# manuelbb-upb/Morbit.jl

Hardware: AMD Instinct MI355X
Metric: RBF build+solve+eval cycles/sec (higher is better)
Workload: dtype f64

## Files before the change

morbit.jl_amd/csrc/backsolve.hip:

```cpp
#include "common.hpp"

namespace mrbf {

namespace bsolve {

constexpr int NB = 128, NTHR = 512;
typedef double v2d __attribute__((ext_vector_type(2)));
typedef double v4d __attribute__((ext_vector_type(4)));
typedef __attribute__((address_space(1))) unsigned gu32;
typedef __attribute__((address_space(1))) double gf64;
typedef __attribute__((address_space(1))) v2d gv2d;

template <int KB>
struct Shared {
    double xs[2][KB][NB];
    int ok;
};

__global__ __launch_bounds__(256) void premul_kernel(const double *__restrict__ L, int64_t lda, const double *__restrict__ linv_all,
                                                     double *__restrict__ Mbuf, int nb, unsigned *__restrict__ flags, int nflags,
                                                     unsigned long long *__restrict__ xb, int nxb) {
    for (int e = blockIdx.x * 256 + threadIdx.x; e < nflags; e += gridDim.x * 256) flags[e] = 0u;
    for (int e = blockIdx.x * 256 + threadIdx.x; e < nxb; e += gridDim.x * 256) xb[e] = ~0ull;
    const int slab = blockIdx.x & 3, t = (blockIdx.x >> 2) & 1, j = blockIdx.x >> 3;
    const int i = j + 1 + t;
    if (i >= nb) return;
    const double *A = L + (int64_t)i * NB + (int64_t)j * NB * lda;
    const double *B = linv_all + (size_t)j * NB * NB;
    double *M = Mbuf + ((size_t)j * 2 + t) * NB * NB;
    const int lane = threadIdx.x & 63, wave = threadIdx.x >> 6, l15 = lane & 15, l4 = lane >> 4;
    const int i0 = 32 * wave, j0 = 32 * slab;
    v4d acc[2][2];
#pragma unroll
    for (int a = 0; a < 2; ++a)
#pragma unroll
        for (int b = 0; b < 2; ++b) acc[a][b] = (v4d){0.0, 0.0, 0.0, 0.0};
    const double *pa = A + (i0 + l15) + (int64_t)(j0 + l4) * lda;
    const double *pb = B + (j0 + l4) + (int64_t)(j0 + l15) * NB;
    constexpr int UK = 8;
    double fa0[2][UK], fa1[2][UK], fb0[2][UK], fb1[2][UK];
    auto burst = [&](int buf) {
#pragma unroll
        for (int u = 0; u < UK; ++u) {
            fa0[buf][u] = pa[(int64_t)4 * u * lda];
            fa1[buf][u] = pa[(int64_t)4 * u * lda + 16];
            fb0[buf][u] = pb[4 * u];
            fb1[buf][u] = pb[4 * u + 16 * NB];
        }
        pa += (int64_t)4 * UK * lda;
        pb += 4 * UK;
    };
    auto mma = [&](int buf) {
#pragma unroll
        for (int u = 0; u < UK; ++u) {
            acc[0][0] = __builtin_amdgcn_mfma_f64_16x16x4f64(fa0[buf][u], fb0[buf][u], acc[0][0], 0, 0, 0);
            acc[0][1] = __builtin_amdgcn_mfma_f64_16x16x4f64(fa0[buf][u], fb1[buf][u], acc[0][1], 0, 0, 0);
            acc[1][0] = __builtin_amdgcn_mfma_f64_16x16x4f64(fa1[buf][u], fb0[buf][u], acc[1][0], 0, 0, 0);
            acc[1][1] = __builtin_amdgcn_mfma_f64_16x16x4f64(fa1[buf][u], fb1[buf][u], acc[1][1], 0, 0, 0);
        }
    };
    const int nburst = (NB - j0) / (4 * UK);
    burst(0);
    for (int b = 0; b < nburst; b += 2) {
        if (b + 1 < nburst) burst(1);
        mma(0);
        if (b + 1 >= nburst) break;
        if (b + 2 < nburst) burst(0);
        mma(1);
    }
#pragma unroll
    for (int a = 0; a < 2; ++a)
#pragma unroll
        for (int b = 0; b < 2; ++b)
#pragma unroll
            for (int r = 0; r < 4; ++r) M[(i0 + 16 * a + l4 + 4 * r) + (size_t)(j0 + 16 * b + l15) * NB] = acc[a][b][r];
}

__device__ __forceinline__ void load_tile(const double *__restrict__ T, int64_t ldt, v2d (&r)[2][8]) {
    const int lane = threadIdx.x & 63, w = threadIdx.x >> 6;
    const double *p = T + (int64_t)(16 * w + 2 * (lane >> 3)) * ldt + 2 * (lane & 7);
#pragma unroll
    for (int cc = 0; cc < 2; ++cc)
#pragma unroll
        for (int u = 0; u < 8; ++u) r[cc][u] = *(const gv2d *)(p + cc * ldt + 16 * u);
}

template <int N>
__device__ __forceinline__ double shl_lanes(double v) {
    const long long b = __double_as_longlong(v);
    const int lo = __builtin_amdgcn_update_dpp((int)b, (int)b, 0x100 + N, 0xf, 0xf, false);
    const int hi = __builtin_amdgcn_update_dpp((int)(b >> 32), (int)(b >> 32), 0x100 + N, 0xf, 0xf, false);
    return __longlong_as_double(((long long)hi << 32) | (unsigned)lo);
}

template <int KB>
__device__ __forceinline__ void tile_dot(const double (*xs)[NB], const v2d (&r)[2][8], double (&out)[2][KB]) {
    const int q = threadIdx.x & 7;
    double acc[2][KB];
#pragma unroll
    for (int cc = 0; cc < 2; ++cc)
#pragma unroll
        for (int l = 0; l < KB; ++l) acc[cc][l] = 0.0;
#pragma unroll
    for (int u = 0; u < 8; ++u) {
#pragma unroll
        for (int l = 0; l < KB; ++l) {
            const v2d x = *(const v2d *)&xs[l][16 * u + 2 * q];
#pragma unroll
            for (int cc = 0; cc < 2; ++cc) acc[cc][l] = fma(r[cc][u][1], x[1], fma(r[cc][u][0], x[0], acc[cc][l]));
        }
    }
#pragma unroll
    for (int cc = 0; cc < 2; ++cc)
#pragma unroll
        for (int l = 0; l < KB; ++l) {
            double v = acc[cc][l];
            v += shl_lanes<4>(v);
            v += shl_lanes<2>(v);
            v += shl_lanes<1>(v);
            out[cc][l] = v;
        }
}

template <int KB>
__device__ __forceinline__ void await_block(Shared<KB> &sh, double (*xs)[NB], const double *glob, int i, double spec, int backoff,
                                            unsigned *abortw, unsigned epoch, unsigned long long spin_ticks, int *status, int code) {
    const int tid = threadIdx.x;
    if (tid >= KB * NB) return;
    const gf64 *src = (const gf64 *)&glob[((size_t)i * KB + tid / NB) * NB + (tid % NB)];
    double v = spec;
    if (__double_as_longlong(v) == -1ll) v = __hip_atomic_load(src, __ATOMIC_RELAXED, __HIP_MEMORY_SCOPE_AGENT);
    unsigned spins = 0;
    unsigned long long t0 = 0;
    while (__double_as_longlong(v) == -1ll) {
        if ((++spins & 63u) == 0u) {
            if (__hip_atomic_load((const gu32 *)abortw, __ATOMIC_RELAXED, __HIP_MEMORY_SCOPE_AGENT) != 0u) {
                sh.ok = 0;
                break;
            }
            const unsigned long long now = wall_clock64();
            if (t0 == 0) t0 = now;
            if (now - t0 > spin_ticks) {
                __hip_atomic_store((gu32 *)abortw, epoch, __ATOMIC_RELAXED, __HIP_MEMORY_SCOPE_AGENT);
                *(__attribute__((address_space(1))) int *)status = code + (i & 0xff);
                sh.ok = 0;
                break;
            }
        }
        for (int b = 0; b < backoff; ++b) __builtin_amdgcn_s_sleep(8);
        v = __hip_atomic_load(src, __ATOMIC_RELAXED, __HIP_MEMORY_SCOPE_AGENT);
    }
    xs[tid / NB][tid % NB] = v;
}

__device__ __forceinline__ void lds_barrier() { asm volatile("s_waitcnt lgkmcnt(0)\n\ts_barrier" ::: "memory"); }

__device__ __forceinline__ void publish(double *dst, v2d v) {
    if (__double_as_longlong(v[0]) == -1ll) v[0] = __longlong_as_double(0x7ff8000000000000ll);
    if (__double_as_longlong(v[1]) == -1ll) v[1] = __longlong_as_double(0x7ff8000000000000ll);
    asm volatile("global_store_dwordx4 %0, %1, off sc1" ::"v"(dst), "v"(v) : "memory");
}

template <int KB>
__global__ __launch_bounds__(NTHR, 1) void backsolve_persistent_kernel(const double *__restrict__ L, int64_t lda, const double *__restrict__ linv_all,
                                                                        const double *__restrict__ Mbuf, double *__restrict__ Y, int64_t ldy, int k0,
                                                                        int nb, unsigned *flags, unsigned epoch, unsigned long long spin_ticks,
                                                                        int *status, int fault, double *__restrict__ xb, double *__restrict__ zb,
                                                                        long long *stamps) {
    __shared__ __attribute__((aligned(16))) Shared<KB> sh;
    const int p = (int)blockIdx.x >> 1;
    const bool finisher = blockIdx.x & 1;
    const int j = nb - 1 - p, tid = threadIdx.x;
    const int lane = tid & 63, col = 16 * (tid >> 6) + 2 * (lane >> 3), q = lane & 7;
    unsigned *abortw = flags + (size_t)nb * 32;
    const int na = nb - 1 - j, npm = na < 2 ? na : 2, npl = na - npm;
    if (tid == 0) sh.ok = 1;
    __syncthreads();
    const double fillv = __longlong_as_double(-1ll);
    if (!finisher) {
        double w[2][KB];
#pragma unroll
        for (int cc = 0; cc < 2; ++cc)
#pragma unroll
            for (int l = 0; l < KB; ++l) w[cc][l] = *(const gf64 *)&Y[(int64_t)(k0 + l) * ldy + (int64_t)j * NB + col + cc];
        const int nst = npl + 1;
        auto fetch = [&](int s, v2d(&r)[2][8]) {
            const double *src = s < npl ? L + (int64_t)(nb - 1 - s) * NB + (int64_t)j * NB * lda : linv_all + (size_t)j * NB * NB;
            load_tile(src, s < npl ? lda : (int64_t)NB, r);
        };
        auto look = [&](int s) {
            const int i = nb - 1 - (s < npl ? s : (npl > 0 ? npl - 1 : 0));
            const int e = tid < KB * NB ? tid : 0;
            return __hip_atomic_load((const gf64 *)&xb[((size_t)i * KB + e / NB) * NB + (e % NB)], __ATOMIC_RELAXED, __HIP_MEMORY_SCOPE_AGENT);
        };
        double spec = fillv, spec2 = fillv;
        auto step = [&](int s, const v2d(&r)[2][8]) -> bool {
            double(*xs)[NB] = sh.xs[s & 1];
            if (s < npl) {
                const int i = nb - 1 - s;
                const int backoff = (i - j - 3) < 24 ? (i - j - 3) : 24;
                await_block<KB>(sh, xs, xb, i, spec, backoff, abortw, epoch, spin_ticks, status, 0x700);
                if (stamps && tid == 0 && s == npl - 1) stamps[256 * 5 + j * 4 + 0] = (long long)wall_clock64();
            } else if (q == 0) {
#pragma unroll
                for (int l = 0; l < KB; ++l) *(v2d *)&xs[l][col] = (v2d){w[0][l], w[1][l]};
            }
            spec = spec2;
            spec2 = look(s + 2);
            if (s + 2 >= npl) spec2 = fillv;
            lds_barrier();
            if (!sh.ok) return false;
            double dsum[2][KB];
            tile_dot<KB>(xs, r, dsum);
#pragma unroll
            for (int cc = 0; cc < 2; ++cc)
#pragma unroll
                for (int l = 0; l < KB; ++l) w[cc][l] = s == npl ? dsum[cc][l] : w[cc][l] - dsum[cc][l];
            return true;
        };
        v2d t0[2][8], t1[2][8], t2[2][8];
        const int o = (3 - nst % 3) % 3, G = (nst + o) / 3;
        if (0 - o >= 0) fetch(0 - o, t0);
        if (1 - o >= 0) fetch(1 - o, t1);
        fetch(2 - o, t2);
        spec = look(0);
        if (npl == 0) spec = fillv;
        spec2 = look(1);
        if (npl <= 1) spec2 = fillv;
        int g = 0;
        if (G >= 2) {
            const int s = -o;
            if (s >= 0 && !step(s, t0)) return;
            fetch(s + 3, t0);
            if (s + 1 >= 0 && !step(s + 1, t1)) return;
            fetch(s + 4, t1);
            if (!step(s + 2, t2)) return;
            fetch(s + 5, t2);
            g = 1;
        }
        for (; g < G - 1; ++g) {
            const int s = 3 * g - o;
            if (!step(s, t0)) return;
            fetch(s + 3, t0);
            if (!step(s + 1, t1)) return;
            fetch(s + 4, t1);
            if (!step(s + 2, t2)) return;
            fetch(s + 5, t2);
        }
        {
            const int s = 3 * (G - 1) - o;
            if (s >= 0 && !step(s, t0)) return;
            if (s + 1 >= 0 && !step(s + 1, t1)) return;
            if (!step(s + 2, t2)) return;
        }
        if (stamps && tid == 0) stamps[256 * 5 + j * 4 + 1] = (long long)wall_clock64();
        if (q == 0) {
#pragma unroll
            for (int l = 0; l < KB; ++l) publish(&zb[((size_t)j * KB + l) * NB + col], (v2d){w[0][l], w[1][l]});
        }
        return;
    }
    v2d tm2[2][8], tm1[2][8];
    if (npm == 2) load_tile(Mbuf + ((size_t)j * 2 + 1) * NB * NB, NB, tm2);
    if (npm >= 1) load_tile(Mbuf + (size_t)j * 2 * NB * NB, NB, tm1);
    double acc[2][KB];
#pragma unroll
    for (int cc = 0; cc < 2; ++cc)
#pragma unroll
        for (int l = 0; l < KB; ++l) acc[cc][l] = 0.0;
    if (npm == 2) {
        await_block<KB>(sh, sh.xs[0], xb, j + 2, fillv, 1, abortw, epoch, spin_ticks, status, 0x700);
        lds_barrier();
        if (!sh.ok) return;
        if (stamps && tid == 0) stamps[256 * 5 + j * 4 + 3] = (long long)wall_clock64();
        tile_dot<KB>(sh.xs[0], tm2, acc);
    }
    v2d zj[KB];
    if (q == 0) {
        unsigned spins = 0;
        unsigned long long t0 = 0;
#pragma unroll
        for (int l = 0; l < KB; ++l) {
            const double *src = &zb[((size_t)j * KB + l) * NB + col];
            while (true) {
                v2d v;
                asm volatile("global_load_dwordx4 %0, %1, off sc1\n\ts_waitcnt vmcnt(0)" : "=v"(v) : "v"(src) : "memory");
                if (__double_as_longlong(v[0]) != -1ll && __double_as_longlong(v[1]) != -1ll) {
                    zj[l] = v;
                    break;
                }
                if ((++spins & 63u) == 0u) {
                    if (__hip_atomic_load((const gu32 *)abortw, __ATOMIC_RELAXED, __HIP_MEMORY_SCOPE_AGENT) != 0u) {
                        sh.ok = 0;
                        break;
                    }
                    const unsigned long long now = wall_clock64();
                    if (t0 == 0) t0 = now;
                    if (now - t0 > spin_ticks) {
                        __hip_atomic_store((gu32 *)abortw, epoch, __ATOMIC_RELAXED, __HIP_MEMORY_SCOPE_AGENT);
                        *(__attribute__((address_space(1))) int *)status = 0x600 + (j & 0xff);
                        sh.ok = 0;
                        break;
                    }
                }
                __builtin_amdgcn_s_sleep(2);
            }
            if (!sh.ok) break;
        }
    }
    if (stamps && tid == 0) stamps[256 * 5 + j * 4 + 2] = (long long)wall_clock64();
    double last[2][KB];
#pragma unroll
    for (int cc = 0; cc < 2; ++cc)
#pragma unroll
        for (int l = 0; l < KB; ++l) last[cc][l] = 0.0;
    if (npm >= 1) {
        if (stamps && tid == 0) stamps[256 * 4 + j] = (long long)wall_clock64();
        await_block<KB>(sh, sh.xs[1], xb, j + 1, fillv, 0, abortw, epoch, spin_ticks, status, 0x700);
        if (stamps && tid == 0) stamps[j * 4 + 0] = (long long)wall_clock64();
        lds_barrier();
        if (!sh.ok) return;
        if (stamps && tid == 0) stamps[j * 4 + 1] = (long long)wall_clock64();
        tile_dot<KB>(sh.xs[1], tm1, last);
    } else {
        lds_barrier();
        if (!sh.ok) return;
    }
    if ((fault & 1) && j == nb / 2) return;
    if (stamps && tid == 0) stamps[j * 4 + 2] = (long long)wall_clock64();
    if (q == 0) {
#pragma unroll
        for (int l = 0; l < KB; ++l) {
            const v2d v = (v2d){(zj[l][0] - acc[0][l]) - last[0][l], (zj[l][1] - acc[1][l]) - last[1][l]};
            publish(&xb[((size_t)j * KB + l) * NB + col], v);
            *(v2d *)&Y[(int64_t)(k0 + l) * ldy + (int64_t)j * NB + col] = v;
        }
    }
}

}

int backsolve_blocked(mrbf_ctx *ctx, int64_t npad, const double *L, int64_t lda, const double *linv_all, double *Y, int64_t ldy, int k);

int backsolve_persistent(mrbf_ctx *ctx, int64_t npad, const double *L, int64_t lda, const double *linv_all, double *Y, int64_t ldy, int k,
                         int *status) {
    using namespace bsolve;
    const int nb = (int)(npad / NB);
    static const int force_old = mrbf_env("MRBF_BACKSOLVE_LAUNCHES") ? atoi(mrbf_env("MRBF_BACKSOLVE_LAUNCHES")) : 0;
    const int ncu = ctx->ncu;
    if (force_old || nb < 3 || nb > ncu || (lda & 1) || (reinterpret_cast<uintptr_t>(L) & 15))
        return backsolve_blocked(ctx, npad, L, lda, linv_all, Y, ldy, k);
    unsigned *flags;
    MRBF_TRY(get_buf(ctx, S_BSOLVE_FLAGS, (size_t)(nb + 1) * 32, &flags));
    const unsigned long long spin_ticks = (unsigned long long)std::max(1, ctx->spin_ms) * 100000ull;
    const int fault = (ctx->debug_fault & 2) ? 1 : 0;
    double *xb, *Mbuf;
    MRBF_TRY(get_buf(ctx, S_BSOLVE_X, (size_t)2 * nb * 4 * NB, &xb));
    MRBF_TRY(get_buf(ctx, S_BSOLVE_M, (size_t)nb * 2 * NB * NB, &Mbuf));
    hipLaunchKernelGGL(premul_kernel, dim3((unsigned)(8 * (nb - 1))), dim3(256), 0, ctx->stream, L, lda, linv_all, Mbuf, nb, flags, (nb + 1) * 32,
                       reinterpret_cast<unsigned long long *>(xb), 2 * nb * 4 * NB);
    static const bool want_stamps = mrbf_env("MRBF_BSOLVE_STAMPS") && atoi(mrbf_env("MRBF_BSOLVE_STAMPS")) != 0;
    long long *stamps = nullptr;
    if (want_stamps) {
        static long long *dbg = nullptr;
        if (!dbg) MRBF_HIP(ctx, hipMalloc(&dbg, (size_t)256 * 9 * sizeof(long long)));
        stamps = dbg;
    }
    unsigned epoch = 0;
    for (int k0 = 0; k0 < k; k0 += 4) {
        const int kb = std::min(4, k - k0);
        ++epoch;
        if (k0 > 0) MRBF_HIP(ctx, hipMemsetAsync(xb, 0xff, (size_t)2 * nb * 4 * NB * sizeof(double), ctx->stream));
#define MRBF_BSP(KBV)                                                                                                          \
    hipLaunchKernelGGL((backsolve_persistent_kernel<KBV>), dim3((unsigned)(2 * nb)), dim3(NTHR), 0, ctx->stream, L, lda, linv_all, Mbuf, Y, ldy, k0, nb, \
                       flags, epoch, spin_ticks, status, fault, xb, xb + (size_t)nb * 4 * NB, stamps)
        if (kb == 1) MRBF_BSP(1); else if (kb == 2) MRBF_BSP(2); else if (kb == 3) MRBF_BSP(3); else MRBF_BSP(4);
#undef MRBF_BSP
    }
    MRBF_HIP(ctx, hipGetLastError());
    if (want_stamps) {
        std::vector<long long> h((size_t)256 * 9);
        MRBF_HIP(ctx, hipMemcpyAsync(h.data(), stamps, h.size() * sizeof(long long), hipMemcpyDeviceToHost, ctx->stream));
        MRBF_HIP(ctx, hipStreamSynchronize(ctx->stream));
        double seen = 0, bar = 0, dot = 0, hop = 0, late = 0;
        int cnt = 0;
        for (int j = 1; j + 2 < nb; ++j) {
            seen += (double)(h[j * 4 + 0] - h[(j + 1) * 4 + 2]);
            bar += (double)(h[j * 4 + 1] - h[j * 4 + 0]);
            dot += (double)(h[j * 4 + 2] - h[j * 4 + 1]);
            hop += (double)(h[j * 4 + 2] - h[(j + 1) * 4 + 2]);
            late += (double)(h[256 * 4 + j] - h[(j + 1) * 4 + 2]);
            ++cnt;
        }
        double a3 = 0, zt = 0, zs = 0, x2 = 0;
        int c2 = 0;
        for (int j = 2; j + 4 < nb; ++j) {
            const long long *S = &h[256 * 5 + j * 4];
            a3 += (double)(S[0] - h[(j + 3) * 4 + 2]);
            zt += (double)(S[1] - S[0]);
            zs += (double)(S[2] - S[1]);
            x2 += (double)(S[3] - h[(j + 2) * 4 + 2]);
            ++c2;
        }
        fprintf(stderr, "[backsolve stamps] streamer: x_{j+3} seen %.2f us after its publication, z_j published %.2f us later, finisher has z_j %.2f us "
                "later; finisher past x_{j+2} %.2f us after that block's publication\n", a3 / c2 / 100.0, zt / c2 / 100.0, zs / c2 / 100.0, x2 / c2 / 100.0);
        fprintf(stderr, "[backsolve stamps] nb %d: publish -> seen %.2f us, seen -> barrier %.2f us, barrier -> publish %.2f us, step %.2f us; "
                "the finisher starts polling %.2f us after the publication\n", nb, seen / cnt / 100.0, bar / cnt / 100.0, dot / cnt / 100.0,
                hop / cnt / 100.0, late / cnt / 100.0);
    }
    return 0;
}

}
```

morbit.jl_amd/csrc/solve.hip:

```cpp
#include "common.hpp"
#include "small.hpp"

namespace mrbf {

__global__ void fit_publish_kernel(const int *__restrict__ dinfo, const double *__restrict__ scal, const unsigned long long *__restrict__ dstat,
                                   int *__restrict__ hflags, double *__restrict__ hscal, unsigned long long *__restrict__ hstat) {
    const int t = threadIdx.x;
    if (t < 4) hflags[t] = dinfo[t];
    if (t >= 4 && t < 6 && scal) hscal[t - 4] = scal[t - 4];
    if (t == 6 && dstat && hstat) hstat[0] = dstat[0];
}

__global__ void fill_saddle_kernel(const double *__restrict__ Pi, int64_t n, int q, double *__restrict__ S, int64_t N) {
    const int64_t idx = (int64_t)blockIdx.x * blockDim.x + threadIdx.x;
    const int64_t tot = n * q;
    if (idx < tot) {
        const int64_t i = idx % n;
        const int t = (int)(idx / n);
        const double v = Pi[idx];
        S[i + (n + t) * N] = v;
        S[(n + t) + i * N] = v;
    } else if (idx < tot + (int64_t)q * q) {
        const int64_t r = idx - tot;
        S[(n + r % q) + (n + r / q) * N] = 0.0;
// ... 223 lines not shown
    MRBF_HIP(ctx, hipEventElapsedTime(&info->ms_solve, ctx->ev[2], ctx->ev[3]));
    return 0;
}

static int fit_small_lu(mrbf_ctx *ctx, mrbf_model *M, const double *Y, mrbf_fit_info *info) {
    smallfit::Prob P;
    double *ws, *scal;
    int *flags;
    MRBF_TRY(get_buf(ctx, S_SMALL_LU, small_lu_scratch_doubles(M->n, M->q), &ws));
    MRBF_TRY(get_buf(ctx, S_SMALL_FLAGS, (size_t)4, &flags));
    MRBF_TRY(get_buf(ctx, S_MISC, (size_t)8, &scal));
    fill_small_prob(ctx, M, Y, ws, flags, scal, nullptr, &P);
    int hflags_local[4] = {0, 0, 0, 0};
    int *hflags = ctx->hpin ? reinterpret_cast<int *>(ctx->hpin + HPIN_SMALL_FLAGS) : hflags_local;
    MRBF_HIP(ctx, hipEventRecord(ctx->ev[0], ctx->stream));
    MRBF_TRY(launch_small_lu(ctx, &P, 1, nullptr));
    MRBF_HIP(ctx, hipEventRecord(ctx->ev[1], ctx->stream));
    MRBF_HIP(ctx, hipMemcpyAsync(hflags, flags, 4 * sizeof(int), hipMemcpyDeviceToHost, ctx->stream));
    MRBF_HIP(ctx, hipStreamSynchronize(ctx->stream));
    info->factor_info = hflags[0];
    info->path = MRBF_PATH_LU;
    if (hflags[0] != 0)
        return fail(ctx, MRBF_ESINGULAR, "saddle matrix is singular (getrf info = %d, N = %lld)", hflags[0], (long long)(M->n + M->q));
    MRBF_HIP(ctx, hipEventElapsedTime(&info->ms_factor, ctx->ev[0], ctx->ev[1]));
    return 0;
}

__global__ void scale_rows_pinv_kernel(double *__restrict__ T, int N, int k, const double *__restrict__ sv) {
    const int idx = blockIdx.x * blockDim.x + threadIdx.x;
    if (idx >= N * k) return;
    const int i = idx % N;
    const double s = sv[i], cut = (double)N * 2.220446049250313e-16 * sv[0];
    T[idx] = (s > cut) ? T[idx] / s : 0.0;
}

static int fit_minnorm(mrbf_ctx *ctx, mrbf_model *M, const double *Y, mrbf_fit_info *info) {
    const int64_t n = M->n, N = n + M->q;
    const int k = M->k, q = M->q;
    const double one = 1.0, zero = 0.0;
    double *S, *B, *Pi, *U, *VT, *sv, *E, *T;
    int *dinfo;
    MRBF_TRY(get_buf(ctx, S_PHI, (size_t)N * N, &S));
    MRBF_TRY(get_buf(ctx, S_RHS, (size_t)N * k, &B));
    MRBF_TRY(get_buf(ctx, S_PI, (size_t)n * q, &Pi));
    MRBF_TRY(get_buf(ctx, S_Q1, (size_t)N * N, &U));
    MRBF_TRY(get_buf(ctx, S_W1, (size_t)N * N, &VT));
    MRBF_TRY(get_buf(ctx, S_TAU, (size_t)2 * N, &sv));
    MRBF_TRY(get_buf(ctx, S_T1, (size_t)N * k, &T));
    MRBF_TRY(get_buf(ctx, S_INFO, (size_t)4, &dinfo));
    E = sv + N;
    hipLaunchKernelGGL(rhs_from_values_kernel, dim3(nblk(N * k)), dim3(256), 0, ctx->stream, Y, n, k, B, N);
    MRBF_HIP(ctx, hipEventRecord(ctx->ev[0], ctx->stream));
    MRBF_TRY(launch_gram(ctx, ctx->gram_mode, M->C, M->Xc, M->sq, n, M->npad, M->d, M->dpad, M->kp, S, N));
    MRBF_HIP(ctx, hipEventRecord(ctx->ev[1], ctx->stream));
    MRBF_TRY(launch_poly_matrix(ctx, M->C, n, M->d, q, Pi, n));
    hipLaunchKernelGGL(fill_saddle_kernel, dim3(nblk(n * q + (int64_t)q * q)), dim3(256), 0, ctx->stream, Pi, n, q, S, N);
    MRBF_HIP(ctx, hipGetLastError());
    MRBF_BLAS(ctx, rocsolver_dgesvd(ctx->blas, rocblas_svect_all, rocblas_svect_all, (int)N, (int)N, S, (int)N, sv, U, (int)N, VT,
                                    (int)N, E, rocblas_outofplace, dinfo));
    MRBF_HIP(ctx, hipEventRecord(ctx->ev[2], ctx->stream));
    int hinfo = 0;
    MRBF_TRY(read_info(ctx, dinfo, &hinfo));
    info->factor_info = hinfo;
    info->path = MRBF_PATH_MINNORM;
    if (hinfo != 0) return fail(ctx, MRBF_ESINGULAR, "SVD of the saddle matrix did not converge (info = %d)", hinfo);
    MRBF_BLAS(ctx, rocblas_dgemm(ctx->blas, rocblas_operation_transpose, rocblas_operation_none, (int)N, k, (int)N, &one, U, (int)N,
                                 B, (int)N, &zero, T, (int)N));
    hipLaunchKernelGGL(scale_rows_pinv_kernel, dim3(nblk(N * k)), dim3(256), 0, ctx->stream, T, (int)N, k, sv);
    MRBF_BLAS(ctx, rocblas_dgemm(ctx->blas, rocblas_operation_transpose, rocblas_operation_none, (int)N, k, (int)N, &one, VT, (int)N,
                                 T, (int)N, &zero, B, (int)N));
    hipLaunchKernelGGL(scatter_solution_kernel, dim3(nblk(M->npad * k + (int64_t)q * k)), dim3(256), 0, ctx->stream, B, N, n,
                       M->npad, k, q, n, M->W, M->Wc, M->lam, B, N);
    MRBF_HIP(ctx, hipGetLastError());
    MRBF_HIP(ctx, hipEventRecord(ctx->ev[3], ctx->stream));
    MRBF_HIP(ctx, hipEventSynchronize(ctx->ev[3]));
    MRBF_HIP(ctx, hipEventElapsedTime(&info->ms_gram, ctx->ev[0], ctx->ev[1]));
    MRBF_HIP(ctx, hipEventElapsedTime(&info->ms_factor, ctx->ev[1], ctx->ev[2]));
    MRBF_HIP(ctx, hipEventElapsedTime(&info->ms_solve, ctx->ev[2], ctx->ev[3]));
    return 0;
}

int backsolve_blocked(mrbf_ctx *ctx, int64_t npad, const double *L, int64_t lda, const double *linv_all, double *Y, int64_t ldy, int k);
int backsolve_persistent(mrbf_ctx *ctx, int64_t npad, const double *L, int64_t lda, const double *linv_all, double *Y, int64_t ldy, int k,
                         int *status);
int launch_update_lower(mrbf_ctx *ctx, const double *A, int64_t lda, const double *B, int64_t ldb, double *C, int64_t ldc, int64_t nt, int K,
                        const double *cvec, double cs, int64_t cn);
int launch_pad_identity(mrbf_ctx *ctx, double *A, int64_t n, int64_t npad, int64_t ld);
int tsmm_tn(mrbf_ctx *ctx, int64_t n, int p, int r, double alpha, const double *A, int64_t lda, const double *B, int64_t ldb, double beta,
            double *C, int64_t ldc);
int symm_panel(mrbf_ctx *ctx, int64_t n, int64_t npad, int q, const double *Phi, int64_t ld, const double *Q, int64_t ldq, double *W,
               int64_t ldwo, bool const_first, double cval);

__global__ void set_rhs_rows_kernel(double *__restrict__ A, int64_t ld, int64_t npad, int xt, const double *__restrict__ B, int k) {
    const int64_t idx = (int64_t)blockIdx.x * blockDim.x + threadIdx.x;
    if (idx >= npad * xt) return;
    const int l = (int)(idx % xt);
    const int64_t i = idx / xt;
    A[(npad + l) + i * ld] = (l < k) ? B[i + (int64_t)l * npad] : 0.0;
}
__global__ void get_rhs_rows_kernel(const double *__restrict__ A, int64_t ld, int64_t npad, double *__restrict__ B, int k) {
    const int64_t idx = (int64_t)blockIdx.x * blockDim.x + threadIdx.x;
    if (idx >= npad * k) return;
    const int l = (int)(idx % k);
    const int64_t i = idx / k;
    B[i + (int64_t)l * npad] = A[(npad + l) + i * ld];
}
__global__ void xc_to_tall_kernel(const double *__restrict__ Xc, int64_t n, int d, int dpad, double *__restrict__ Tall, int64_t lt,
                                  int64_t dq) {
    const int64_t idx = (int64_t)blockIdx.x * blockDim.x + threadIdx.x;
    if (idx >= n * d) return;
    const int64_t i = idx / d;
    const int t = (int)(idx % d);
    Tall[(dq + i) + (int64_t)t * lt] = Xc[i * dpad + t];
}
__global__ void build_q1_kernel(const double *__restrict__ Tall, int64_t lt, int64_t dq, int64_t n, int64_t npad, int q,
                                double *__restrict__ Q1) {
    const int64_t idx = (int64_t)blockIdx.x * blockDim.x + threadIdx.x;
    if (idx >= npad * q) return;
    const int64_t i = idx % npad;
    const int t = (int)(idx / npad);
    double v = 0.0;
    if (i < n) v = (t == 0) ? 1.0 / sqrt((double)n) : Tall[(dq + i) + (int64_t)(t - 1) * lt];
    Q1[idx] = v;
}
__global__ void shift_from_trace_kernel(double *__restrict__ scal, double nphi0, double nmq, int *__restrict__ flags) {
    const double mu = (nphi0 - scal[0]) / nmq;
    const bool ok = mu > 0.0 && mu < 1e300;
    scal[1] = ok ? mu : 1.0;
    flags[2] = ok ? 0 : 1;
}

__global__ void build_panels_kernel(const double *__restrict__ Q1, const double *__restrict__ W, const double *__restrict__ scal,
                                    int64_t n, int64_t npad, int q, int K2, int skip, double *__restrict__ PA, double *__restrict__ PB,
                                    double *__restrict__ v0) {
    const int64_t idx = (int64_t)blockIdx.x * blockDim.x + threadIdx.x;
    if (idx >= npad * K2) return;
    const double mu = scal[1];
    const int64_t i = idx % npad;
    const int t = (int)(idx / npad);
    const int qq = q - skip;
    double a = 0.0, b = 0.0;
    if (i < n && t < 2 * qq) {
        const int tt = t % qq + skip;
        const double qv = Q1[i + (int64_t)tt * npad];
        const double vv = fma(-0.5 * mu, qv, W[i + (int64_t)tt * npad]);
        a = (t < qq) ? qv : vv;
        b = (t < qq) ? vv : qv;
    }
    PA[idx] = a;
    PB[idx] = b;
    if (skip && t == 0) v0[i] = (i < n) ? fma(-0.5 * mu, Q1[i], W[i]) : 0.0;
}
__global__ __launch_bounds__(64) void finish_lambda_kernel(double *__restrict__ T1, int q, int k, double sqrtn, const double *__restrict__ mean) {
    __shared__ double part[64];
    const int l = blockIdx.x, tid = threadIdx.x;
    if (l >= k) return;
    double acc = 0.0;
    for (int t = 1 + tid; t < q; t += 64) acc = fma(mean[t - 1], T1[t + (int64_t)l * q], acc);
    part[tid] = acc;
    __syncthreads();
    if (tid == 0) {
        double dsum = 0.0;
        for (int u = 0; u < 64; ++u) dsum += part[u];
        T1[(int64_t)l * q] = T1[(int64_t)l * q] / sqrtn - dsum;
    }
}

// ... 239 lines not shown
        if (tailq) {
            double *scratch;
            MRBF_TRY(get_buf(ctx, S_PI, tail_basis_scratch_doubles(), &scratch));
            MRBF_TRY(get_buf(ctx, S_QR_INV, (size_t)128 * 128, &LxInv));
            MRBF_TRY(launch_tail_basis(ctx, M, Y, scratch, LxInv, T1, Q1, B, builtin ? Phi : nullptr, ld, xt, dinfo));
        } else if (q > 1) {
            dq = round_up(d, 128);
            lt = dq + npad;
            MRBF_TRY(get_buf(ctx, S_PI, (size_t)lt * dq, &Tall));
            MRBF_HIP(ctx, hipMemsetAsync(Tall, 0, (size_t)lt * dq * sizeof(double), ctx->stream));
            hipLaunchKernelGGL(xc_to_tall_kernel, dim3(nblk(n * d)), dim3(256), 0, ctx->stream, M->Xc, n, d, M->dpad, Tall, lt, dq);
            MRBF_TRY(tsmm_tn(ctx, n, d, d, 1.0, Tall + dq, lt, Tall + dq, lt, 0.0, Tall, lt));
            MRBF_TRY(launch_pad_identity(ctx, Tall, d, dq, lt));
            if (dq == 128) MRBF_TRY(get_buf(ctx, S_QR_INV, (size_t)128 * 128, &LxInv));
            MRBF_TRY(potrf_blocked_tall(ctx, dq, lt, Tall, lt, dinfo + 1, LxInv, popt));
        }
        if (!tailq) hipLaunchKernelGGL(build_q1_kernel, dim3(nblk(npad * q)), dim3(256), 0, ctx->stream, Tall, lt, dq, n, npad, q, Q1);
        if (!fused) MRBF_HIP(ctx, hipMemsetAsync(Wm, 0, (size_t)npad * q * sizeof(double), ctx->stream));
        if (!tailq) {
            MRBF_TRY(tsmm_tn(ctx, n, q, k, 1.0, Q1, npad, B, npad, 0.0, T1, q));
            hipLaunchKernelGGL(sub_qt_kernel, dim3((unsigned)((n + 63) / 64)), dim3(256), 0, ctx->stream, B, npad, Q1, npad, T1, n, q, k);
            if (builtin) hipLaunchKernelGGL(set_rhs_rows_kernel, dim3(nblk(npad * xt)), dim3(256), 0, ctx->stream, Phi, ld, npad, xt, B, k);
        }
        if (side) MRBF_HIP(ctx, hipEventRecord(ctx->evx[1], ctx->stream));
    }
    ctx->stream = main_stream;
    MRBF_HIP(ctx, hipEventRecord(ctx->ev[0], ctx->stream));
    double *Wpart = nullptr, *rspart = nullptr;
    int nseg = 0;
    if (fused)
        MRBF_TRY(launch_gram_w(ctx, M, Phi, ld, &Wpart, &rspart, &nseg));
    else
        MRBF_TRY(launch_gram(ctx, ctx->gram_mode, M->C, M->Xc, M->sq, n, M->npad, M->d, M->dpad, M->kp, Phi, ld));
    MRBF_HIP(ctx, hipEventRecord(ctx->ev[1], ctx->stream));
    if (side) MRBF_HIP(ctx, hipStreamWaitEvent(ctx->stream, ctx->evx[1], 0));
    if (fused) {
        const int skip = (q > 1 && round_up(2 * (q - 1), 16) < round_up(2 * q, 16)) ? 1 : 0;
        const int K2 = (int)round_up(2 * (q - skip), 16);
        double *PA, *PB, *v0 = nullptr;
        MRBF_TRY(get_buf(ctx, S_STAGE_C, (size_t)npad * K2, &PA));
        MRBF_TRY(get_buf(ctx, S_STAGE_D, (size_t)npad * K2, &PB));
        if (skip) MRBF_TRY(get_buf(ctx, S_V0, (size_t)npad, &v0));
        MRBF_TRY(launch_projection_small(ctx, M, Wpart, rspart, nseg, LxInv, Q1, Wm, G, scal, dinfo, K2, skip, PA, PB, v0));
        MRBF_TRY(launch_update_lower(ctx, PA, npad, PB, npad, Phi, ld, npad / 128, K2, v0, 1.0 / std::sqrt((double)n), n));
    } else if (q > 0) {
        MRBF_TRY(symm_panel(ctx, n, npad, q, Phi, ld, Q1, npad, Wm, npad, true, 1.0 / std::sqrt((double)n)));
        MRBF_TRY(tsmm_tn(ctx, n, q, q, 1.0, Q1, npad, Wm, npad, 0.0, G, q));
        hipLaunchKernelGGL(trace_kernel, dim3(1), dim3(256), 0, ctx->stream, G, q, scal);
        MRBF_BLAS(ctx, rocblas_dgemm(ctx->blas, rocblas_operation_none, rocblas_operation_none, (int)n, q, q, &mhalf, Q1, (int)npad,
                                     G, q, &one, Wm, (int)npad));
        hipLaunchKernelGGL(shift_from_trace_kernel, dim3(1), dim3(1), 0, ctx->stream, scal, (double)n * M->kp.phi0,
                           (double)std::max<int64_t>(n - q, 1), dinfo);
        const int skip = (q > 1 && round_up(2 * (q - 1), 16) < round_up(2 * q, 16)) ? 1 : 0;
        const int K2 = (int)round_up(2 * (q - skip), 16);
        double *PA, *PB, *v0 = nullptr;
        MRBF_TRY(get_buf(ctx, S_STAGE_C, (size_t)npad * K2, &PA));
        MRBF_TRY(get_buf(ctx, S_STAGE_D, (size_t)npad * K2, &PB));
        if (skip) MRBF_TRY(get_buf(ctx, S_V0, (size_t)npad, &v0));
        hipLaunchKernelGGL(build_panels_kernel, dim3(nblk(npad * K2)), dim3(256), 0, ctx->stream, Q1, Wm, scal, n, npad, q, K2, skip, PA, PB, v0);
        MRBF_TRY(launch_update_lower(ctx, PA, npad, PB, npad, Phi, ld, npad / 128, K2, v0, 1.0 / std::sqrt((double)n), n));
    }
    MRBF_HIP(ctx, hipEventRecord(ctx->ev[2], ctx->stream));
    int hinfo = 0;
    double *linv_all = nullptr;
    if (builtin) {
        MRBF_TRY(get_buf(ctx, S_CHOL_WS, (size_t)npad * 128, &linv_all));
        MRBF_TRY(launch_pad_identity(ctx, Phi, n, npad, ld));
        if (q == 0) hipLaunchKernelGGL(set_rhs_rows_kernel, dim3(nblk(npad * xt)), dim3(256), 0, ctx->stream, Phi, ld, npad, xt, B, k);
        popt.xreal = k;
        popt.info_clean = true;
        MRBF_TRY(potrf_blocked_tall(ctx, npad, npad + xt, Phi, ld, dinfo, linv_all, popt));
        MRBF_HIP(ctx, hipEventRecord(ctx->ev[3], ctx->stream));
    } else {
        int *dpot;
        MRBF_TRY(get_buf(ctx, S_IPIV, (size_t)4, &dpot));
        MRBF_BLAS(ctx, rocsolver_dpotrf(ctx->blas, rocblas_fill_lower, (int)n, Phi, (int)ld, dpot));
        MRBF_HIP(ctx, hipMemcpyAsync(dinfo, dpot, sizeof(int), hipMemcpyDeviceToDevice, ctx->stream));
        MRBF_HIP(ctx, hipEventRecord(ctx->ev[3], ctx->stream));
    }
    double *T1w = nullptr;
    if (q > 0) MRBF_TRY(get_buf(ctx, S_T1W, (size_t)q * k, &T1w));
    auto solve_tail = [&](bool persistent) -> int {
        if (builtin) {
            hipLaunchKernelGGL(get_rhs_rows_kernel, dim3(nblk(npad * k)), dim3(256), 0, ctx->stream, Phi, ld, npad, B, k);
            if (persistent)
                MRBF_TRY(backsolve_persistent(ctx, npad, Phi, ld, linv_all, B, npad, k, dinfo + 3));
            else
                MRBF_TRY(backsolve_blocked(ctx, npad, Phi, ld, linv_all, B, npad, k));
        } else {
            MRBF_BLAS(ctx, rocsolver_dpotrs(ctx->blas, rocblas_fill_lower, (int)n, k, Phi, (int)ld, B, (int)npad));
        }
        static const int tail3 = mrbf_env("MRBF_TAIL3") ? atoi(mrbf_env("MRBF_TAIL3")) : 1;
        if (tail3 && q > 0 && q <= 129 && k <= 16 && (q == 1 || LxInv)) {
            const int nch = (int)(npad / 64);
            double *T2, *part;
            MRBF_TRY(get_buf(ctx, S_T2, (size_t)q * k, &T2));
            MRBF_TRY(get_buf(ctx, S_TAIL_PART, (size_t)nch * 2 * k * q, &part));
            hipLaunchKernelGGL(tail_dots_kernel, dim3((unsigned)nch), dim3(256), 0, ctx->stream, B, npad, Q1, Wm, npad, n, q, k, part);
            hipLaunchKernelGGL(tail_coeff_kernel, dim3(1), dim3(1024), 0, ctx->stream, part, nch, q, k, q > 1 ? d : 0, T1, G, fused ? 1.0 : 0.5, LxInv,
                               std::sqrt((double)n), M->mean, T2, T1w);
            hipLaunchKernelGGL(tail_apply_kernel, dim3((unsigned)nch), dim3(256), 0, ctx->stream, B, npad, Q1, npad, T2, T1w, n, M->npad, q, k, M->W,
                               M->Wc, M->lam);
            MRBF_HIP(ctx, hipGetLastError());
            return 0;
        }
        if (q > 0) {
            double *T2;
            MRBF_TRY(get_buf(ctx, S_T2, (size_t)q * k, &T2));
            MRBF_HIP(ctx, hipMemcpyAsync(T1w, T1, (size_t)q * k * sizeof(double), hipMemcpyDeviceToDevice, ctx->stream));
            MRBF_TRY(tsmm_tn(ctx, n, q, k, 1.0, Q1, npad, B, npad, 0.0, T2, q));
            hipLaunchKernelGGL(sub_qt_kernel, dim3((unsigned)((n + 63) / 64)), dim3(256), 0, ctx->stream, B, npad, Q1, npad, T2, n, q, k);
            MRBF_TRY(tsmm_tn(ctx, n, q, k, -1.0, Wm, npad, B, npad, 1.0, T1w, q));
            if (q > 1) {
                if (LxInv)
                    hipLaunchKernelGGL(apply_linv_t_kernel, dim3(1), dim3(256), 0, ctx->stream, LxInv, d, T1w + 1, (int64_t)q, k);
                else if (d <= 256)
                    hipLaunchKernelGGL(trsm_lt_small_kernel, dim3(1), dim3(256), 0, ctx->stream, Tall, lt, d, T1w + 1, (int64_t)q, k);
                else
                    MRBF_BLAS(ctx, rocblas_dtrsm(ctx->blas, rocblas_side_left, rocblas_fill_lower, rocblas_operation_transpose,
                                                 rocblas_diagonal_non_unit, d, k, &one, Tall, (int)lt, T1w + 1, q));
            }
            hipLaunchKernelGGL(finish_lambda_kernel, dim3((unsigned)k), dim3(64), 0, ctx->stream, T1w, q, k, std::sqrt((double)n), M->mean);
        }
        hipLaunchKernelGGL(scatter_solution_kernel, dim3(nblk(M->npad * k + (int64_t)q * k)), dim3(256), 0, ctx->stream, B, npad, n,
                           M->npad, k, q, (int64_t)0, M->W, M->Wc, M->lam, T1w ? T1w : B, (int64_t)q);
        MRBF_HIP(ctx, hipGetLastError());
        return 0;
    };
    MRBF_TRY(solve_tail(true));
    MRBF_HIP(ctx, hipEventRecord(ctx->ev[4], ctx->stream));
    {
        int hflags_local[4] = {0, 0, 0, 0};
        double hscal_local[2] = {0.0, 0.0};
        int *hflags = ctx->hpin ? reinterpret_cast<int *>(ctx->hpin + HPIN_FIT_FLAGS) : hflags_local;
        double *hscal = ctx->hpin ? reinterpret_cast<double *>(ctx->hpin + HPIN_FIT_SCAL) : hscal_local;
        hscal[0] = hscal[1] = 0.0;
        static const int publish = mrbf_env("MRBF_FIT_PUBLISH") ? atoi(mrbf_env("MRBF_FIT_PUBLISH")) : 1;
        if (ctx->hpin && publish) {
            unsigned long long *hstat = nullptr;
            const unsigned long long *dstat = nullptr;
            if (ctx->mega_stat_pending && ctx->mega_stat_dev) {
                ctx->hpin[HPIN_MEGA_STAT] = ~0ull;
                hstat = &ctx->hpin[HPIN_MEGA_STAT];
                dstat = ctx->mega_stat_dev;
                ctx->mega_stat_pending = 2;
            }
            hipLaunchKernelGGL(fit_publish_kernel, dim3(1), dim3(64), 0, ctx->stream, (const int *)dinfo, q > 0 ? (const double *)scal : nullptr, dstat,
                               hflags, hscal, hstat);
        } else {
        MRBF_HIP(ctx, hipMemcpyAsync(hflags, dinfo, 4 * sizeof(int), hipMemcpyDeviceToHost, ctx->stream));
        if (q > 0) MRBF_HIP(ctx, hipMemcpyAsync(hscal, scal, 2 * sizeof(double), hipMemcpyDeviceToHost, ctx->stream));
        MRBF_TRY(mega_stat_enqueue(ctx));
        }
        MRBF_HIP(ctx, hipStreamSynchronize(ctx->stream));
        MRBF_TRY(mega_stat_finish(ctx));
        info->ms_factor_device = ctx->last_device_ms;
        hinfo = hflags[0];
        if (hinfo < 0) {
            *gave_up = 1;
            info->giveup_code = -hinfo;
            return 0;
        }
        info->factor_info = hinfo;
        if (q > 0) info->mu = hscal[1];
        if (hflags[1] < 0) {
            *gave_up = 1;
            info->giveup_code = -hflags[1];
            return 0;
        }
        if (hflags[1] != 0) {
            *not_pd = 1;
// ... 249 lines not shown
```

Measured before the change: 175.9.

## Fold premultiply into persistent backsolve and merge RHS copy with flag reset

The separate premul kernel is removed. Its L·Linv products are now computed by extra producer blocks inside the first persistent backsolve launch, and consumers wait on per-block ready counters before loading M with coherent loads. The first few head blocks (nhead) skip the M shortcut entirely so the chain can start before any products exist. The RHS row copy is fused with the flag and xb reset into one prep kernel, which drops a launch. The cost is a grid with many more blocks, added spin-waits on producer flags, and atomic stores and loads for M.

```diff
diff --git a/morbit.jl_amd/csrc/backsolve.hip b/morbit.jl_amd/csrc/backsolve.hip
--- a/morbit.jl_amd/csrc/backsolve.hip
+++ b/morbit.jl_amd/csrc/backsolve.hip
@@ -17,18 +17,13 @@
     int ok;
 };
 
-__global__ __launch_bounds__(256) void premul_kernel(const double *__restrict__ L, int64_t lda, const double *__restrict__ linv_all,
-                                                     double *__restrict__ Mbuf, int nb, unsigned *__restrict__ flags, int nflags,
-                                                     unsigned long long *__restrict__ xb, int nxb) {
-    for (int e = blockIdx.x * 256 + threadIdx.x; e < nflags; e += gridDim.x * 256) flags[e] = 0u;
-    for (int e = blockIdx.x * 256 + threadIdx.x; e < nxb; e += gridDim.x * 256) xb[e] = ~0ull;
-    const int slab = blockIdx.x & 3, t = (blockIdx.x >> 2) & 1, j = blockIdx.x >> 3;
+__device__ __forceinline__ void premul_slab(const double *__restrict__ L, int64_t lda, const double *__restrict__ linv_all, double *Mbuf, int j,
+                                            int t, int slab, int t4) {
     const int i = j + 1 + t;
-    if (i >= nb) return;
     const double *A = L + (int64_t)i * NB + (int64_t)j * NB * lda;
     const double *B = linv_all + (size_t)j * NB * NB;
     double *M = Mbuf + ((size_t)j * 2 + t) * NB * NB;
-    const int lane = threadIdx.x & 63, wave = threadIdx.x >> 6, l15 = lane & 15, l4 = lane >> 4;
+    const int lane = t4 & 63, wave = t4 >> 6, l15 = lane & 15, l4 = lane >> 4;
     const int i0 = 32 * wave, j0 = 32 * slab;
     v4d acc[2][2];
 #pragma unroll
@@ -73,7 +68,21 @@
 #pragma unroll
         for (int b = 0; b < 2; ++b)
 #pragma unroll
-            for (int r = 0; r < 4; ++r) M[(i0 + 16 * a + l4 + 4 * r) + (size_t)(j0 + 16 * b + l15) * NB] = acc[a][b][r];
+            for (int r = 0; r < 4; ++r)
+                __hip_atomic_store((gf64 *)&M[(i0 + 16 * a + l4 + 4 * r) + (size_t)(j0 + 16 * b + l15) * NB], acc[a][b][r], __ATOMIC_RELAXED,
+                                   __HIP_MEMORY_SCOPE_AGENT);
+}
+
+__global__ __launch_bounds__(256) void get_rhs_rows_prep_kernel(const double *__restrict__ A, int64_t ld, int64_t npad, double *__restrict__ B, int64_t ldb, int k,
+                                                            unsigned *__restrict__ flags, int nflags, unsigned long long *__restrict__ xb,
+                                                            int nxb) {
+    for (int e = blockIdx.x * 256 + threadIdx.x; e < nflags; e += gridDim.x * 256) flags[e] = 0u;
+    for (int e = blockIdx.x * 256 + threadIdx.x; e < nxb; e += gridDim.x * 256) xb[e] = ~0ull;
+    const int64_t idx = (int64_t)blockIdx.x * 256 + threadIdx.x;
+    if (!A || idx >= npad * k) return;
+    const int l = (int)(idx % k);
+    const int64_t i = idx / k;
+    B[i + (int64_t)l * ldb] = A[(npad + l) + i * ld];
 }
 
 __device__ __forceinline__ void load_tile(const double *__restrict__ T, int64_t ldt, v2d (&r)[2][8]) {
@@ -83,6 +92,17 @@
     for (int cc = 0; cc < 2; ++cc)
 #pragma unroll
         for (int u = 0; u < 8; ++u) r[cc][u] = *(const gv2d *)(p + cc * ldt + 16 * u);
+}
+
+__device__ __forceinline__ void load_tile_sc1(const double *T, v2d (&r)[2][8]) {
+    const int lane = threadIdx.x & 63, w = threadIdx.x >> 6;
+    const gf64 *p = (const gf64 *)(T + (size_t)(16 * w + 2 * (lane >> 3)) * NB + 2 * (lane & 7));
+#pragma unroll
+    for (int cc = 0; cc < 2; ++cc)
+#pragma unroll
+        for (int u = 0; u < 8; ++u)
+            r[cc][u] = (v2d){__hip_atomic_load(p + cc * NB + 16 * u, __ATOMIC_RELAXED, __HIP_MEMORY_SCOPE_AGENT),
+                             __hip_atomic_load(p + cc * NB + 16 * u + 1, __ATOMIC_RELAXED, __HIP_MEMORY_SCOPE_AGENT)};
 }
 
 template <int N>
@@ -153,6 +173,30 @@
     xs[tid / NB][tid % NB] = v;
 }
 
+template <int KB>
+__device__ __forceinline__ void await_products(Shared<KB> &sh, const unsigned *ready, int j, unsigned *abortw, unsigned epoch,
+                                               unsigned long long spin_ticks, int *status) {
+    unsigned spins = 0;
+    unsigned long long t0 = 0;
+    while (__hip_atomic_load((const gu32 *)ready, __ATOMIC_RELAXED, __HIP_MEMORY_SCOPE_AGENT) < 4u) {
+        if ((++spins & 63u) == 0u) {
+            if (__hip_atomic_load((const gu32 *)abortw, __ATOMIC_RELAXED, __HIP_MEMORY_SCOPE_AGENT) != 0u) {
+                sh.ok = 0;
+                break;
+            }
+            const unsigned long long now = wall_clock64();
+            if (t0 == 0) t0 = now;
+            if (now - t0 > spin_ticks) {
+                __hip_atomic_store((gu32 *)abortw, epoch, __ATOMIC_RELAXED, __HIP_MEMORY_SCOPE_AGENT);
+                *(__attribute__((address_space(1))) int *)status = 0x500 + (j & 0xff);
+                sh.ok = 0;
+                break;
+            }
+        }
+        __builtin_amdgcn_s_sleep(2);
+    }
+}
+
 __device__ __forceinline__ void lds_barrier() { asm volatile("s_waitcnt lgkmcnt(0)\n\ts_barrier" ::: "memory"); }
 
 __device__ __forceinline__ void publish(double *dst, v2d v) {
@@ -163,17 +207,31 @@
 
 template <int KB>
 __global__ __launch_bounds__(NTHR, 1) void backsolve_persistent_kernel(const double *__restrict__ L, int64_t lda, const double *__restrict__ linv_all,
-                                                                        const double *__restrict__ Mbuf, double *__restrict__ Y, int64_t ldy, int k0,
-                                                                        int nb, unsigned *flags, unsigned epoch, unsigned long long spin_ticks,
+                                                                        double *Mbuf, double *__restrict__ Y, int64_t ldy, int k0, int nb, int nhead,
+                                                                        int nprod, unsigned *flags, unsigned epoch, unsigned long long spin_ticks,
                                                                         int *status, int fault, double *__restrict__ xb, double *__restrict__ zb,
                                                                         long long *stamps) {
     __shared__ __attribute__((aligned(16))) Shared<KB> sh;
-    const int p = (int)blockIdx.x >> 1;
-    const bool finisher = blockIdx.x & 1;
+    const int bid = (int)blockIdx.x;
+    if (bid >= 2 * nhead && bid < 2 * nhead + nprod) {
+        const int pb = bid - 2 * nhead;
+        const int c = pb >> 2, t = (pb >> 1) & 1, h = pb & 1, jp = nb - 1 - nhead - c;
+        const int half = (int)threadIdx.x >> 8;
+        if (jp + 1 + t < nb) premul_slab(L, lda, linv_all, Mbuf, jp, t, half ? 3 - h : h, (int)threadIdx.x & 255);
+        asm volatile("s_waitcnt vmcnt(0)" ::: "memory");
+        __syncthreads();
+        if (threadIdx.x == 0) __hip_atomic_fetch_add((gu32 *)&flags[(size_t)jp * 32], 1u, __ATOMIC_RELAXED, __HIP_MEMORY_SCOPE_AGENT);
+        return;
+    }
+    const int cb = bid < 2 * nhead ? bid : bid - nprod;
+    const int p = cb >> 1;
+    const bool finisher = cb & 1;
     const int j = nb - 1 - p, tid = threadIdx.x;
+    if (finisher && p < nhead) return;
+
     const int lane = tid & 63, col = 16 * (tid >> 6) + 2 * (lane >> 3), q = lane & 7;
     unsigned *abortw = flags + (size_t)nb * 32;
-    const int na = nb - 1 - j, npm = na < 2 ? na : 2, npl = na - npm;
+    const int na = nb - 1 - j, npm = p < nhead ? 0 : 2, npl = na - npm;
     if (tid == 0) sh.ok = 1;
     __syncthreads();
     const double fillv = __longlong_as_double(-1ll);
@@ -254,6 +312,19 @@
             if (!step(s + 2, t2)) return;
         }
         if (stamps && tid == 0) stamps[256 * 5 + j * 4 + 1] = (long long)wall_clock64();
+        if (npm == 0) {
+            if ((fault & 1) && j == nb / 2) return;
+            if (stamps && tid == 0) stamps[j * 4 + 2] = (long long)wall_clock64();
+            if (q == 0) {
+#pragma unroll
+                for (int l = 0; l < KB; ++l) {
+                    const v2d v = (v2d){w[0][l], w[1][l]};
+                    publish(&xb[((size_t)j * KB + l) * NB + col], v);
+                    *(v2d *)&Y[(int64_t)(k0 + l) * ldy + (int64_t)j * NB + col] = v;
+                }
+            }
+            return;
+        }
         if (q == 0) {
 #pragma unroll
             for (int l = 0; l < KB; ++l) publish(&zb[((size_t)j * KB + l) * NB + col], (v2d){w[0][l], w[1][l]});
@@ -261,8 +332,17 @@
         return;
     }
     v2d tm2[2][8], tm1[2][8];
-    if (npm == 2) load_tile(Mbuf + ((size_t)j * 2 + 1) * NB * NB, NB, tm2);
-    if (npm >= 1) load_tile(Mbuf + (size_t)j * 2 * NB * NB, NB, tm1);
+    {
+        if (tid == 0) {
+            if (stamps) stamps[256 * 9 + j] = (long long)wall_clock64();
+            await_products<KB>(sh, flags + (size_t)j * 32, j, abortw, epoch, spin_ticks, status);
+            if (stamps) stamps[256 * 10 + j] = (long long)wall_clock64();
+        }
+        __syncthreads();
+        if (!sh.ok) return;
+        load_tile_sc1(Mbuf + ((size_t)j * 2 + 1) * NB * NB, tm2);
+        load_tile_sc1(Mbuf + (size_t)j * 2 * NB * NB, tm1);
+    }
     double acc[2][KB];
 #pragma unroll
     for (int cc = 0; cc < 2; ++cc)
@@ -343,13 +423,18 @@
 int backsolve_blocked(mrbf_ctx *ctx, int64_t npad, const double *L, int64_t lda, const double *linv_all, double *Y, int64_t ldy, int k);
 
 int backsolve_persistent(mrbf_ctx *ctx, int64_t npad, const double *L, int64_t lda, const double *linv_all, double *Y, int64_t ldy, int k,
-                         int *status) {
+                         int *status, bool rhs_rows) {
     using namespace bsolve;
     const int nb = (int)(npad / NB);
     static const int force_old = mrbf_env("MRBF_BACKSOLVE_LAUNCHES") ? atoi(mrbf_env("MRBF_BACKSOLVE_LAUNCHES")) : 0;
+    const unsigned ncopy = rhs_rows ? (unsigned)((npad * k + 255) / 256) : 0u;
     const int ncu = ctx->ncu;
-    if (force_old || nb < 3 || nb > ncu || (lda & 1) || (reinterpret_cast<uintptr_t>(L) & 15))
+    if (force_old || nb < 3 || nb > ncu || (lda & 1) || (reinterpret_cast<uintptr_t>(L) & 15)) {
+        if (rhs_rows)
+            hipLaunchKernelGGL(get_rhs_rows_prep_kernel, dim3(ncopy), dim3(256), 0, ctx->stream, L, lda, npad, Y, ldy, k, (unsigned *)nullptr, 0,
+                               (unsigned long long *)nullptr, 0);
         return backsolve_blocked(ctx, npad, L, lda, linv_all, Y, ldy, k);
+    }
     unsigned *flags;
     MRBF_TRY(get_buf(ctx, S_BSOLVE_FLAGS, (size_t)(nb + 1) * 32, &flags));
     const unsigned long long spin_ticks = (unsigned long long)std::max(1, ctx->spin_ms) * 100000ull;
@@ -357,56 +442,82 @@
     double *xb, *Mbuf;
     MRBF_TRY(get_buf(ctx, S_BSOLVE_X, (size_t)2 * nb * 4 * NB, &xb));
     MRBF_TRY(get_buf(ctx, S_BSOLVE_M, (size_t)nb * 2 * NB * NB, &Mbuf));
-    hipLaunchKernelGGL(premul_kernel, dim3((unsigned)(8 * (nb - 1))), dim3(256), 0, ctx->stream, L, lda, linv_all, Mbuf, nb, flags, (nb + 1) * 32,
-                       reinterpret_cast<unsigned long long *>(xb), 2 * nb * 4 * NB);
+    hipLaunchKernelGGL(get_rhs_rows_prep_kernel, dim3(std::max(ncopy, 32u)), dim3(256), 0, ctx->stream, rhs_rows ? L : nullptr, lda, npad, Y, ldy, k,
+                       flags, (nb + 1) * 32, reinterpret_cast<unsigned long long *>(xb), 2 * nb * 4 * NB);
+
     static const bool want_stamps = mrbf_env("MRBF_BSOLVE_STAMPS") && atoi(mrbf_env("MRBF_BSOLVE_STAMPS")) != 0;
     long long *stamps = nullptr;
     if (want_stamps) {
         static long long *dbg = nullptr;
-        if (!dbg) MRBF_HIP(ctx, hipMalloc(&dbg, (size_t)256 * 9 * sizeof(long long)));
+        if (!dbg) MRBF_HIP(ctx, hipMalloc(&dbg, (size_t)256 * 11 * sizeof(long long)));
         stamps = dbg;
     }
+    const int nhead = std::max(2, std::min(8, nb / 2));
     unsigned epoch = 0;
     for (int k0 = 0; k0 < k; k0 += 4) {
         const int kb = std::min(4, k - k0);
         ++epoch;
+        const int nprod = k0 == 0 ? 4 * (nb - nhead) : 0;
         if (k0 > 0) MRBF_HIP(ctx, hipMemsetAsync(xb, 0xff, (size_t)2 * nb * 4 * NB * sizeof(double), ctx->stream));
 #define MRBF_BSP(KBV)                                                                                                          \
-    hipLaunchKernelGGL((backsolve_persistent_kernel<KBV>), dim3((unsigned)(2 * nb)), dim3(NTHR), 0, ctx->stream, L, lda, linv_all, Mbuf, Y, ldy, k0, nb, \
-                       flags, epoch, spin_ticks, status, fault, xb, xb + (size_t)nb * 4 * NB, stamps)
+    hipLaunchKernelGGL((backsolve_persistent_kernel<KBV>), dim3((unsigned)(nprod + 2 * nb)), dim3(NTHR), 0, ctx->stream, L, lda, linv_all, Mbuf, Y, ldy, k0, nb, \
+                       nhead, nprod, flags, epoch, spin_ticks, status, fault, xb, xb + (size_t)nb * 4 * NB, stamps)
         if (kb == 1) MRBF_BSP(1); else if (kb == 2) MRBF_BSP(2); else if (kb == 3) MRBF_BSP(3); else MRBF_BSP(4);
 #undef MRBF_BSP
     }
     MRBF_HIP(ctx, hipGetLastError());
     if (want_stamps) {
-        std::vector<long long> h((size_t)256 * 9);
+        std::vector<long long> h((size_t)256 * 11);
         MRBF_HIP(ctx, hipMemcpyAsync(h.data(), stamps, h.size() * sizeof(long long), hipMemcpyDeviceToHost, ctx->stream));
         MRBF_HIP(ctx, hipStreamSynchronize(ctx->stream));
+        const int jl = nb - 1 - nhead;
+        const auto pub = [&](int j) { return h[j * 4 + 2]; };
         double seen = 0, bar = 0, dot = 0, hop = 0, late = 0;
         int cnt = 0;
-        for (int j = 1; j + 2 < nb; ++j) {
-            seen += (double)(h[j * 4 + 0] - h[(j + 1) * 4 + 2]);
+        for (int j = 1; j <= jl; ++j) {
+            seen += (double)(h[j * 4 + 0] - pub(j + 1));
             bar += (double)(h[j * 4 + 1] - h[j * 4 + 0]);
-            dot += (double)(h[j * 4 + 2] - h[j * 4 + 1]);
-            hop += (double)(h[j * 4 + 2] - h[(j + 1) * 4 + 2]);
-            late += (double)(h[256 * 4 + j] - h[(j + 1) * 4 + 2]);
+            dot += (double)(pub(j) - h[j * 4 + 1]);
+            hop += (double)(pub(j) - pub(j + 1));
+            late += (double)(h[256 * 4 + j] - pub(j + 1));
             ++cnt;
         }
         double a3 = 0, zt = 0, zs = 0, x2 = 0;
         int c2 = 0;
-        for (int j = 2; j + 4 < nb; ++j) {
+        for (int j = 2; j <= jl && j + 3 < nb; ++j) {
             const long long *S = &h[256 * 5 + j * 4];
-            a3 += (double)(S[0] - h[(j + 3) * 4 + 2]);
+            a3 += (double)(S[0] - pub(j + 3));
             zt += (double)(S[1] - S[0]);
             zs += (double)(S[2] - S[1]);
-            x2 += (double)(S[3] - h[(j + 2) * 4 + 2]);
+            x2 += (double)(S[3] - pub(j + 2));
             ++c2;
         }
-        fprintf(stderr, "[backsolve stamps] streamer: x_{j+3} seen %.2f us after its publication, z_j published %.2f us later, finisher has z_j %.2f us "
-                "later; finisher past x_{j+2} %.2f us after that block's publication\n", a3 / c2 / 100.0, zt / c2 / 100.0, zs / c2 / 100.0, x2 / c2 / 100.0);
-        fprintf(stderr, "[backsolve stamps] nb %d: publish -> seen %.2f us, seen -> barrier %.2f us, barrier -> publish %.2f us, step %.2f us; "
-                "the finisher starts polling %.2f us after the publication\n", nb, seen / cnt / 100.0, bar / cnt / 100.0, dot / cnt / 100.0,
-                hop / cnt / 100.0, late / cnt / 100.0);
+        double mw = 0, ms = 0, mworst = 1e300;
+        for (int j = 0; j <= jl; ++j) {
+            mw += (double)(h[256 * 10 + j] - h[256 * 9 + j]);
+            const double slack = (double)(h[j * 4 + 0] - h[256 * 10 + j]);
+            ms += slack;
+            mworst = std::min(mworst, slack);
+        }
+        fprintf(stderr, "[backsolve stamps] nb %d, head %d: head step %.2f us; M-ready wait: mean %.2f us, ended %.2f us (mean) / %.2f us (least) before "
+                "x_{j+1} was seen\n", nb, nhead, (double)(pub(jl + 1) - pub(nb - 1)) / (nhead - 1) / 100.0, mw / (jl + 1) / 100.0, ms / (jl + 1) / 100.0,
+                mworst / 100.0);
+        {
+            double qs[4];
+            for (int f = 0; f < 4; ++f) {
+                const int hi = jl + 1 - f * (jl + 1) / 4, lo = jl + 1 - (f + 1) * (jl + 1) / 4;
+                qs[f] = hi > lo ? (double)(pub(lo) - pub(hi)) / (hi - lo) / 100.0 : 0.0;
+            }
+            fprintf(stderr, "[backsolve stamps] chain: first publication to last %.2f us; step by quarter of the chain behind the head %.2f %.2f %.2f %.2f us\n",
+                    (double)(pub(0) - pub(nb - 1)) / 100.0, qs[0], qs[1], qs[2], qs[3]);
+        }
+        if (c2 > 0)
+            fprintf(stderr, "[backsolve stamps] streamer: x_{j+3} seen %.2f us after its publication, z_j published %.2f us later, finisher has z_j %.2f us "
+                    "later; finisher past x_{j+2} %.2f us after that block's publication\n", a3 / c2 / 100.0, zt / c2 / 100.0, zs / c2 / 100.0, x2 / c2 / 100.0);
+        if (cnt > 0)
+            fprintf(stderr, "[backsolve stamps] publish -> seen %.2f us, seen -> barrier %.2f us, barrier -> publish %.2f us, step %.2f us; "
+                    "the finisher starts polling %.2f us after the publication\n", seen / cnt / 100.0, bar / cnt / 100.0, dot / cnt / 100.0,
+                    hop / cnt / 100.0, late / cnt / 100.0);
     }
     return 0;
 }
diff --git a/morbit.jl_amd/csrc/solve.hip b/morbit.jl_amd/csrc/solve.hip
--- a/morbit.jl_amd/csrc/solve.hip
+++ b/morbit.jl_amd/csrc/solve.hip
@@ -329,7 +329,7 @@
 
 int backsolve_blocked(mrbf_ctx *ctx, int64_t npad, const double *L, int64_t lda, const double *linv_all, double *Y, int64_t ldy, int k);
 int backsolve_persistent(mrbf_ctx *ctx, int64_t npad, const double *L, int64_t lda, const double *linv_all, double *Y, int64_t ldy, int k,
-                         int *status);
+                         int *status, bool rhs_rows);
 int launch_update_lower(mrbf_ctx *ctx, const double *A, int64_t lda, const double *B, int64_t ldb, double *C, int64_t ldc, int64_t nt, int K,
                         const double *cvec, double cs, int64_t cn);
 int launch_pad_identity(mrbf_ctx *ctx, double *A, int64_t n, int64_t npad, int64_t ld);
@@ -735,11 +735,12 @@
     if (q > 0) MRBF_TRY(get_buf(ctx, S_T1W, (size_t)q * k, &T1w));
     auto solve_tail = [&](bool persistent) -> int {
         if (builtin) {
-            hipLaunchKernelGGL(get_rhs_rows_kernel, dim3(nblk(npad * k)), dim3(256), 0, ctx->stream, Phi, ld, npad, B, k);
-            if (persistent)
-                MRBF_TRY(backsolve_persistent(ctx, npad, Phi, ld, linv_all, B, npad, k, dinfo + 3));
-            else
+            if (persistent) {
+                MRBF_TRY(backsolve_persistent(ctx, npad, Phi, ld, linv_all, B, npad, k, dinfo + 3, true));
+            } else {
+                hipLaunchKernelGGL(get_rhs_rows_kernel, dim3(nblk(npad * k)), dim3(256), 0, ctx->stream, Phi, ld, npad, B, k);
                 MRBF_TRY(backsolve_blocked(ctx, npad, Phi, ld, linv_all, B, npad, k));
+            }
         } else {
             MRBF_BLAS(ctx, rocsolver_dpotrs(ctx->blas, rocblas_fill_lower, (int)n, k, Phi, (int)ld, B, (int)npad));
         }
```

Result: no change. 177.0 (median of 6 runs) (+0.6%).
